# AkshayThiru/incentive-design-mpc

Hardware: AMD Instinct MI355X
Metric: LoMPC QP solves/sec (higher is better)
Workload: dtype f64

## Files before the change

incentive-design-mpc_amd/csrc/lompc_ctx.hpp:

```cpp
#pragma once
#include <hip/hip_runtime.h>
#include <stdint.h>

#include <algorithm>
#include <string>
#include <vector>

#include "lompc_qp.hpp"
#include "../../include/lompc_amd.h"

#define NPX 7
enum {
  PX_COST = 0,
  PX_PRICE0 = 1,
  PX_MAX_ERR = 2,
  PX_N_OK = 3,
  PX_N_REPAIRED = 4,
  PX_N_FAILED = 5,
  PX_N_INVALID = 6
};

struct lompc_ctx {
  int device = 0;
  int N = 0;
// ... 66 lines not shown
  int scalar_cells = 0;
  int nblk = 0;
  int n_cu = 0;
  bool close = false;
  bool close_no_w = true;
  int* d_arrive = nullptr;
  int n_empty = 0;
  CtxEnds ce{};
  int eval_occ = 1;
  int64_t eval_occ_key = -1;
  int64_t cap_S = 0, cap_blk = 0, cap_cells = 0;
  const double* gamma = nullptr;
  const double* w_ref = nullptr;
  double* d_stats_own = nullptr;
  double* d_stats = nullptr;
  int64_t* d_set_off = nullptr;
  int* d_blk_prefix = nullptr;
  int4* d_blk = nullptr;
  double* d_window = nullptr;
  unsigned long long* d_wacc = nullptr;
  double* d_partial = nullptr;
  int* d_fail_cnt = nullptr;
  int* d_fail_idx = nullptr;
  int* t_cnt = nullptr;
  double* t_lo = nullptr;
  double* t_ge = nullptr;
  double* t_cf = nullptr;
  double2* t_ab = nullptr;
  uint8_t* t_sl = nullptr;
  uint8_t* d_ws = nullptr;
  struct Stepped {
    bool ok = false;
    int nblk = 0, np_wg = 0;
    char* d_map = nullptr;
    char* h_map = nullptr;
    int64_t cap_map = 0;
    PathTab tab[2]{};
    uint8_t* sl3 = nullptr;
    int64_t cap_cells = 0;
    double* part[2] = {nullptr, nullptr};
    int* fcnt[2] = {nullptr, nullptr};
    int* fidx[2] = {nullptr, nullptr};
    int64_t cap_blk = 0;
    int occ = 0;
    int64_t occ_key = -1;
    bool wide = false;
    bool stg = false;
    PathTab wt{};
    int64_t cap_wt = 0;
    double* rpart = nullptr;
    int* rfcnt = nullptr;
    int* rfidx = nullptr;
    int64_t cap_rrec = 0;
  } stp;
  int* d_errflag = nullptr;
  unsigned long long* d_tally = nullptr;
  struct lompc_comm* comm = nullptr;
  double* d_xsend = nullptr;
  double* d_xrecv = nullptr;
  int64_t cap_xsend = 0, cap_xrecv = 0;
  const int* skip = nullptr;
  int* d_loop = nullptr;
  struct lq_host_loop* h_loop = nullptr;
  double* h_dec = nullptr;
  int cap_loop_iter = 0;
  double* d_aggrec = nullptr;
  int64_t cap_aggrec = 0;
  int64_t aggrec_zero = -1;
  bool sorted = false;
  int nsblk = 0, aggF = 0;
  int4* d_sblk = nullptr;
  int* d_sblk_prefix = nullptr;
  unsigned long long* d_bsum = nullptr;
  unsigned long long* d_P = nullptr;
  int* d_pos = nullptr;
  int4* d_sinfo = nullptr;
  int64_t cap_sblk = 0, cap_P = 0, cap_pos = 0, cap_sinfo = 0;
  char* h_buf = nullptr;
  int64_t cap_h = 0;
  int64_t reserve_B = 0;
  int64_t h_off_at = 0;
  hipEvent_t ev_stage = nullptr;
  int prof = 0;
  std::vector<hipEvent_t> prof_ev[LOMPC_PLAN_KERNELS], prof_pool;
  std::vector<int> prof_mult[LOMPC_PLAN_KERNELS];
  double prof_ms[LOMPC_PLAN_KERNELS] = {0.0, 0.0, 0.0, 0.0};
  int64_t prof_n[LOMPC_PLAN_KERNELS] = {0, 0, 0, 0};
  std::string err;
};

#define HIPCHK(obj, call)                                                        \
  do {                                                                           \
    hipError_t e__ = (call);                                                     \
    if (e__ != hipSuccess) {                                                     \
      if (obj) (obj)->err = std::string(#call) + ": " + hipGetErrorString(e__); \
      return LOMPC_ERR_HIP;                                                      \
    }                                                                            \
  } while (0)

template <typename O>
static inline int fail_arg(O* o, const char* msg) {
  if (o) o->err = msg;
  return LOMPC_ERR_INVALID_ARG;
}

template <typename O, typename T>
// ... 44 lines not shown
```

incentive-design-mpc_amd/csrc/lompc_plan.hip:

```cpp
#include <hip/hip_ext.h>
#include <hip/hip_runtime.h>
#include <stdint.h>
#include <string.h>

#include <algorithm>
#include <chrono>
#include <cmath>
#include <cstdlib>
#include <map>
#include <mutex>
#include <type_traits>
#include <utility>

#include "lompc_ctx.hpp"
#include "lompc_loopstep.hpp"
#include "lompc_wave.hpp"

#ifdef LOMPC_STAMPS
#ifdef LOMPC_STAMPS_RT
#define __builtin_amdgcn_s_memtime __builtin_amdgcn_s_memrealtime
#endif
__device__ long long g_stamps[65536 * 8];
__device__ long long g_wstart[32768 * 8];
__device__ unsigned long long g_lstamps[64 * 16];
// ... 1594 lines not shown
#if LQ_EVALS_KARGS
    typedef __attribute__((address_space(4))) const EvalArgs karg_t;
    typedef __attribute__((address_space(4))) const EvalsArgs kargx_t;
    typedef __attribute__((address_space(4))) const char kargc_t;
    karg_t* ka = (karg_t*)__builtin_amdgcn_kernarg_segment_ptr();
    asm volatile("" : "+s"(ka));
    const EvalArgs& ar = *(const EvalArgs*)ka;
    const EvalsArgs& x = *(const EvalsArgs*)(kargx_t*)((kargc_t*)ka + KARG_X);
#else
    const EvalArgs& ar = a;
    const EvalsArgs& x = x_;
#endif
    const int j = x.run0 + r;
    RunOff ro;
    ro.tab = (int64_t)(j % x.slots) * x.SG;
    ro.rec = r * x.nblk;
    ro.ev = (int64_t)j * x.ev_stride;
    ro.lmbd = ar.lmbd + (size_t)j * x.lm_stride;
    ro.lmbd_r = ar.lmbd_r + (size_t)j * x.lr_stride;
    ro.launder = true;
    ro.gamma_lds = r > 0;
    ro.pipelined = LQ_EVALS_PIPELINED;
    ro.first = r == 0;
#ifdef LQ_EVALS_NOSTAGE
    ro.nostage = r > 0;
#endif
    int bl = b;
    asm volatile("" : "+s"(bl));
#ifdef LOMPC_STAMPS
    const long long t0__ = __builtin_amdgcn_s_memtime();
#endif
    eval_block<NT, false>(ar, bl, nullptr, ro);
#if LQ_EVALS_RUN_BARRIER
    __syncthreads();
#endif
#ifdef LOMPC_STAMPS
    if (threadIdx.x == 0 && r < 32 && b < 512) {
      long long* q = g_stamps + ((size_t)b * 32 + r) * 8;
      const long long* e = g_stamps + (32768 + b) * 8;
      q[0] = t0__;
      q[1] = e[6];
      q[2] = e[0];
      q[3] = e[2];
      q[4] = e[3];
      q[5] = e[1];
      q[6] = e[4];
      q[7] = __builtin_amdgcn_s_memtime();
    }
#endif
  }
}

template <int NT>
__global__ __launch_bounds__(EVAL_EVS, EVAL_MIN_WAVES) void k_evals_st(EvalArgs a, EvalsArgs x) {
  extern __shared__ __attribute__((aligned(16))) double2 s_dyn[];
  const int b = (int)blockIdx.x, tid = (int)threadIdx.x, lane = tid & 63;
  const int wv = __builtin_amdgcn_readfirstlane(tid >> 6);
  const int N = NT ? NT : a.N, G = a.G, capc = a.cap;
  const size_t tb = ctab_bytes(N, G, capc);
  char* const base = reinterpret_cast<char*>(s_dyn);
  double* const accw = reinterpret_cast<double*>(base + 2 * tb);
  double* const red = accw + (size_t)2 * EVAL_WAVES * N;
  const int s = a.blk[b].x;
  if (wv == LQ_EVALS_RW) {
    const int NS = eval_row_stride(N);
    for (int k = 0; k < 2; ++k) {
      const CTab T = ctab_at(base + k * tb, N, G, capc);
      for (int i = lane; i < 2 * NS; i += 64) T.ab[(size_t)capc * NS + i] = make_double2(0.0, 0.0);
      for (int i = lane; i < N; i += 64) accw[((size_t)k * EVAL_WAVES + LQ_EVALS_RW) * N + i] = 0.0;
      if (lane < 8) red[((size_t)k * EVAL_WAVES + LQ_EVALS_RW) * 8 + lane] = 0.0;
    }
    stage_compact(a, s, (int64_t)(x.run0 % x.slots) * x.SG, ctab_at(base, N, G, capc), N, G, capc, lane);
  }
  __syncthreads();
  for (int r = 0; r < x.nruns; ++r) {
    const int j = x.run0 + r;
    if (wv < LQ_EVALS_RW) {
      RunOff ro;
      ro.tab = (int64_t)(j % x.slots) * x.SG;
      ro.rec = r * x.nblk;
      ro.ev = (int64_t)j * x.ev_stride;
      ro.lmbd = a.lmbd + (size_t)j * x.lm_stride;
      ro.lmbd_r = a.lmbd_r + (size_t)j * x.lr_stride;
      ro.launder = true;
      ro.gamma_lds = r > 0;
      ro.buf = r & 1;
      int bl = b;
      asm volatile("" : "+s"(bl));
      eval_block<NT, false, true>(a, bl, nullptr, ro);
    } else if (r + 1 < x.nruns) {
      stage_compact(a, s, (int64_t)((j + 1) % x.slots) * x.SG, ctab_at(base + ((r + 1) & 1) * tb, N, G, capc), N, G,
                    capc, lane);
    }
    __syncthreads();
    if (wv == 0) {
      const int rb = r * x.nblk + b;
      const int par = r & 1;
      double* part = a.partial + (size_t)rb * (N + NPX);
      for (int c = lane; c < N + NPX; c += 64) {
        double v = 0.0;
        if (c < N) {
          for (int k = 0; k < EVAL_WAVES; ++k) v += accw[((size_t)par * EVAL_WAVES + k) * N + c];
        } else {
          const int xx = c - N;
          for (int k = 0; k < EVAL_WAVES; ++k) {
            const double u = red[((size_t)par * EVAL_WAVES + k) * 8 + xx];
            v = xx == PX_MAX_ERR ? fmax(v, u) : v + u;
          }
        }
        st_wt8(part + c, v);
      }
      if (lane == 0) st_wt4(a.fail_cnt + (size_t)rb * EVAL_WAVES + LQ_EVALS_RW, 0);
    }
  }
}

typedef void (*EvalsKernel)(EvalArgs, EvalsArgs);
EvalsKernel evals_st_kernel(int N) {
  switch (N) {
    case 12: return k_evals_st<12>;
    case 16: return k_evals_st<16>;
    case 24: return k_evals_st<24>;
    case 48: return k_evals_st<48>;
    default: return k_evals_st<0>;
  }
}
EvalsKernel evals_kernel(int N) {
  switch (N) {
    case 12: return k_evals<12>;
    case 16: return k_evals<16>;
    case 24: return k_evals<24>;
    case 48: return k_evals<48>;
    default: return k_evals<0>;
  }
}

struct ClosesArgs {
  int run0, nruns, slots, nblk, S, last;
  int rel;
  int64_t lm_stride, lr_stride, ev_stride, sw_stride, st_stride, SG;
};

__global__ __launch_bounds__(256) void k_closes(FinalArgs f, ClosesArgs x) {
  __shared__ double red[LQ_FIN_CLASSES][FIN_W];
  __shared__ double rep[LQ_FIN_CLASSES][FIN_W];
  const int r = (int)blockIdx.x / x.S, s = (int)blockIdx.x - r * x.S, j = x.run0 + r, N = f.N;
  FinalArgs c = f;
  c.lmbd = f.lmbd + (size_t)j * x.lm_stride;
  c.lmbd_r = f.lmbd_r + (size_t)j * x.lr_stride;
  c.t_sl = f.t_sl + (int64_t)(j % x.slots) * x.SG * 64;
  c.partial = f.partial + (size_t)r * x.nblk * (N + NPX);
  c.fail_cnt = f.fail_cnt + (size_t)r * x.nblk * EVAL_WAVES;
  c.fail_idx = f.fail_idx + (size_t)r * x.nblk * EVAL_MAXB;
  const bool last = j == x.last;
  if (x.ev_stride) {
    const size_t eo = (size_t)j * x.ev_stride;
    if (f.w) c.w = f.w + eo * N;
    if (f.cost) c.cost = f.cost + eo;
    if (f.w0) c.w0 = f.w0 + eo;
    if (f.status) c.status = f.status + eo;
  } else if (!last) {
    c.w = c.cost = c.w0 = nullptr;
    c.status = nullptr;
  }
  const int js = x.rel ? r : j;
  if (f.set_sum_w) c.set_sum_w = (x.sw_stride || last) ? f.set_sum_w + (size_t)js * x.sw_stride : nullptr;
  if (f.set_stats) c.set_stats = (x.st_stride || last) ? f.set_stats + (size_t)js * x.st_stride : nullptr;
  if (!last) c.stats = nullptr;
  finalize_set<4, false>(c, s, red, rep);
}

#include "lompc_agg.hpp"
#include "lompc_scalar.hpp"

constexpr int LQ_LOOP_G = 16;
constexpr int LQ_LOOP_G2 = 32;

// ... 1330 lines not shown
  const int64_t rounds = std::max<int64_t>(1, (10 * B + 9ll * slots * maxb - 1) / (9ll * slots * maxb));
  const int64_t target = free1 + (rounds - 1) * slots;
  std::vector<int64_t> off(S + 1);
  {
    const int64_t* hoff = reinterpret_cast<const int64_t*>(p->h_buf + p->h_off_at);
    for (int64_t s = 0; s <= S; ++s) off[s] = hoff[s];
  }
  std::vector<int4> blks;
  std::vector<int> pre;
  block_map(off.data(), S, B, maxb, target, p->n_cu, wide && rounds == 1, blks, pre);
  int64_t nblk = (int64_t)blks.size();
  const size_t o_pre = ((size_t)nblk * sizeof(int4) + 15) & ~(size_t)15;
  const size_t bytes = o_pre + (size_t)(S + 1) * sizeof(int);
  int rc;
  if ((int64_t)bytes > z.cap_map) {
    if (z.h_map) HIPCHK(p, hipHostFree(z.h_map));
    z.h_map = nullptr;
    HIPCHK(p, hipHostMalloc((void**)&z.h_map, bytes, hipHostMallocDefault));
    if ((rc = grow(p, &z.d_map, bytes))) return rc;
    z.cap_map = (int64_t)bytes;
  }
  HIPCHK(p, hipStreamSynchronize(st));
  memcpy(z.h_map, blks.data(), (size_t)nblk * sizeof(int4));
  memcpy(z.h_map + o_pre, pre.data(), (size_t)(S + 1) * sizeof(int));
  HIPCHK(p, hipMemcpyAsync(z.d_map, z.h_map, bytes, hipMemcpyHostToDevice, st));
  z.nblk = (int)nblk;
  if (ncell > z.cap_cells) {
    for (int k = 0; k < 2; ++k) {
      auto& t = z.tab[k];
      if ((rc = grow(p, &t.cnt, ncell)) || (rc = grow(p, &t.lo, ncell)) || (rc = grow(p, &t.ge, ncell * LQ_PPL)) ||
          (rc = grow(p, &t.cf, ncell * LQ_PPL * 8)) || (rc = grow(p, &t.ab, ncell * LQ_PPL * N)))
        return rc;
    }
    if ((rc = grow(p, &z.sl3, 3 * (size_t)ncell * 64))) return rc;
    z.cap_cells = ncell;
  }
  if (nblk > z.cap_blk) {
    for (int k = 0; k < 2; ++k)
      if ((rc = grow(p, &z.part[k], (size_t)nblk * (N + NPX))) || (rc = grow(p, &z.fcnt[k], (size_t)nblk * EVAL_WAVES)) ||
          (rc = grow(p, &z.fidx[k], (size_t)nblk * EVAL_MAXB)))
        return rc;
    z.cap_blk = nblk;
  }
  z.ok = true;
  z.wide = wide;
  z.stg = stg;
  return LOMPC_OK;
}

#ifndef LQ_WIDE_RUNS
#define LQ_WIDE_RUNS 64
#endif
#define LQ_WIDE_BYTES (1ll << 30)

int64_t wide_fit(const lompc_plan* p) {
  const int64_t ncell = p->S * p->G;
  const int64_t cell_bytes = LQ_PPL * (16 * (int64_t)p->N + 8 * 8 + 8) + 4 + 8 + 64;
  return std::min<int64_t>(LQ_WIDE_BYTES / (ncell * cell_bytes), INT32_MAX / 64 / ncell) - 1;
}

int wide_ring(lompc_plan* p, hipStream_t st) {
  auto& z = p->stp;
  int rc;
  const int N = p->N;
  const int64_t ncell = p->S * p->G;
  const int64_t ring = (std::min<int64_t>(LQ_WIDE_RUNS, wide_fit(p)) + 1) * ncell;
  if (ring > z.cap_wt) {
    auto& t = z.wt;
    const int64_t c = ring;
    if ((rc = grow(p, &t.cnt, c)) || (rc = grow(p, &t.lo, c)) || (rc = grow(p, &t.ge, c * LQ_PPL)) ||
        (rc = grow(p, &t.cf, c * LQ_PPL * 8)) || (rc = grow(p, &t.ab, c * LQ_PPL * N)) || (rc = grow(p, &t.sl, c * 64)))
      return rc;
    HIPCHK(p, hipMemsetAsync(t.ge, 0, (size_t)c * LQ_PPL * sizeof(*t.ge), st));
    HIPCHK(p, hipMemsetAsync(t.cf, 0, (size_t)c * LQ_PPL * 8 * sizeof(*t.cf), st));
    HIPCHK(p, hipMemsetAsync(t.ab, 0, (size_t)c * LQ_PPL * N * sizeof(*t.ab), st));
    HIPCHK(p, hipMemsetAsync(t.sl, 0, (size_t)c * 64 * sizeof(*t.sl), st));
    z.cap_wt = c;
  }
  return LOMPC_OK;
}

int lq_run_steps_stepped(lompc_plan* p, const double* lmbd, int64_t lmbd_stride, const double* lmbd_r,
                         int64_t lmbd_r_stride, int n_runs, int profile_every, bool span_events, double* w, double* cost,
                         double* w0, int8_t* status, int64_t ev_stride, double* set_sum_w, int64_t sw_stride,
                         double* set_stats, int64_t st_stride, bool split, hipStream_t st, bool scalar = false) {
  auto& z = p->stp;
  int rc;
  const int N = p->N;
  const int64_t ncell = p->S * p->G, L = p->S * (N + LOMPC_SET_STATS);
  const int K = n_runs;
  const int64_t fit = wide_fit(p);
  const int Kc = (int)std::min<int64_t>({(int64_t)K, LQ_WIDE_RUNS, fit});
  const bool wide = (p->flags & LOMPC_PLAN_WARM_START) == 0 && Kc >= 1;
  const int slots = Kc + 1;
  if ((!z.ok || z.wide != wide || z.stg != (wide && evals_stg_ok(p))) && (rc = stepped_setup(p, st, wide))) return rc;
  const bool xr = p->comm != nullptr;
  if (xr && (rc = lq_xbufs(p, 2))) return rc;
  if (wide && (rc = wide_ring(p, st))) return rc;
  auto tab = [&](int j) {
    if (wide) {
      const int64_t o = (int64_t)(j % slots) * ncell;
      PathTab t;
      t.cnt = z.wt.cnt + o;
      t.lo = z.wt.lo + o;
      t.ge = z.wt.ge + o * LQ_PPL;
      t.cf = z.wt.cf + o * LQ_PPL * 8;
      t.ab = z.wt.ab + o * LQ_PPL * N;
      t.sl = z.wt.sl + o * 64;
      return t;
    }
    PathTab t = z.tab[j & 1];
    t.sl = z.sl3 + (size_t)(j % 3) * ncell * 64;
    return t;
  };
  auto lm = [&](int j) { return lmbd + (size_t)j * lmbd_stride; };
  auto lr = [&](int j) { return lmbd_r + (size_t)j * lmbd_r_stride; };
  auto sw_of = [&](int j) { return set_sum_w ? set_sum_w + (size_t)j * sw_stride : nullptr; };
  auto st_of = [&](int j) { return set_stats ? set_stats + (size_t)j * st_stride : nullptr; };
  auto xsend = [&](int j) { return p->d_xsend + (size_t)(j & 1) * L; };
// ... 1 lines not shown
    const size_t eo = (size_t)j * ev_stride;
    eval_args(p, lm(j), lr(j), w ? w + eo * N : nullptr, cost ? cost + eo : nullptr, w0 ? w0 + eo : nullptr,
              status ? status + eo : nullptr, tab(j), a, r);
    a.blk = reinterpret_cast<const int4*>(z.d_map);
    a.nblk = z.nblk;
    a.partial = z.part[j & 1];
    r.partial = z.part[j & 1];
    a.fail_cnt = z.fcnt[j & 1];
    r.fail_cnt = z.fcnt[j & 1];
    a.fail_idx = z.fidx[j & 1];
    r.fail_idx = z.fidx[j & 1];
    r.blk_prefix = reinterpret_cast<const int*>(z.d_map + (((size_t)z.nblk * sizeof(int4) + 15) & ~(size_t)15));
    r.set_sum_w = xr ? xsend(j) : sw_of(j);
    r.set_stats = xr ? xsend(j) + p->S * N : st_of(j);
    if (ev_stride == 0 && j != K - 1) {
      r.w = r.cost = r.w0 = nullptr;
      r.status = nullptr;
    }
  };
  const size_t lds = eval_lds(N, p->G, p->cap);
  const StepKernel kern = step_kernel(N);
  if (wide && (!split || z.stg || !w)) {
    const int64_t rec_run = (int64_t)z.nblk * ((N + NPX) * 8 + EVAL_WAVES * 4 + EVAL_MAXB * 4);
    const int64_t kr = std::max<int64_t>(1, std::min<int64_t>(std::min<int64_t>(LQ_WIDE_RUNS, fit), LQ_WIDE_BYTES / rec_run));
    const int64_t need = kr * z.nblk;
    if (need > z.cap_rrec) {
      if ((rc = grow(p, &z.rpart, need * (N + NPX))) || (rc = grow(p, &z.rfcnt, need * EVAL_WAVES)) ||
          (rc = grow(p, &z.rfidx, need * EVAL_MAXB)))
        return rc;
      HIPCHK(p, hipMemsetAsync(z.rpart, 0, (size_t)need * (N + NPX) * sizeof(*z.rpart), st));
      HIPCHK(p, hipMemsetAsync(z.rfcnt, 0, (size_t)need * EVAL_WAVES * sizeof(*z.rfcnt), st));
      HIPCHK(p, hipMemsetAsync(z.rfidx, 0, (size_t)need * EVAL_MAXB * sizeof(*z.rfidx), st));
      z.cap_rrec = need;
    }
    if (xr && (rc = lq_xbufs(p, Kc, Kc))) return rc;
    EvalArgs ea;
    FinalArgs ff;
    eval_args(p, lmbd, lmbd_r, w, cost, w0, status, tab(0), ea, ff);
    ea.piece_sums = w ? 0 : 1;
    ea.blk = reinterpret_cast<const int4*>(z.d_map);
    ea.nblk = z.nblk;
    ea.partial = z.rpart;
    ff.partial = z.rpart;
    ea.fail_cnt = z.rfcnt;
    ff.fail_cnt = z.rfcnt;
    ea.fail_idx = z.rfidx;
    ff.fail_idx = z.rfidx;
    ff.blk_prefix = reinterpret_cast<const int*>(z.d_map + (((size_t)z.nblk * sizeof(int4) + 15) & ~(size_t)15));
    ff.set_sum_w = xr ? p->d_xsend : set_sum_w;
    ff.set_stats = xr ? p->d_xsend + p->S * N : set_stats;
    const int grp = split ? 1 : (int)std::min<int64_t>(Kc, kr);
    if (z.stg) ea.cap = std::min(LQ_EVALS_CAP, p->G * LQ_PPL);
    const size_t lds_e = z.stg ? evals_st_lds(N, p->G, ea.cap) : lds;
    for (int g0 = 0; g0 < K; g0 += grp) {
      const int n = std::min(grp, K - g0);
      {
        PathArgs pw = path_args(p, lmbd, lmbd_r, z.wt);
        hipEvent_t e0 = nullptr, e1 = nullptr;
        if (plan_prof_begin(p, LOMPC_PLAN_K_PATH, &e0, &e1)) return fail_arg(p, "profiling events");
        hipExtLaunchKernelGGL(paths_kernel(N), dim3((unsigned)(n * ncell)), dim3(64), 0, st, e0, e1, 0, pw, lmbd_stride,
                              lmbd_r_stride, g0, slots);
        HIPCHK(p, hipGetLastError());
        plan_prof_end(p, LOMPC_PLAN_K_PATH, e0, e1, scalar ? n : 1);
      }
      {
        hipEvent_t e0 = nullptr, e1 = nullptr;
        const bool ev = !span_events || g0 == 0;
        const int kk = scalar ? LOMPC_PLAN_K_SCALAR : LOMPC_PLAN_K_EVAL;
        if (ev && plan_prof_begin(p, kk, &e0, &e1)) return fail_arg(p, "profiling events");
        const EvalsArgs x{g0, n, slots, z.nblk, lmbd_stride, lmbd_r_stride, ev_stride, ncell};
        if (scalar)
          hipExtLaunchKernelGGL(k_scalars, dim3((unsigned)(n * z.nblk)), dim3(EVAL_EVS), scalar_lds(p->G, p->scalar_cells), st,
                                e0, e1, 0, ea, x, p->scalar_cells, K - 1);
        else
          hipExtLaunchKernelGGL(z.stg ? evals_st_kernel(N) : evals_kernel(N), dim3((unsigned)z.nblk), dim3(EVAL_EVS), lds_e, st,
                                e0, e1, 0, ea, x);
        HIPCHK(p, hipGetLastError());
        if (ev) plan_prof_end(p, kk, e0, e1, n);
      }
      {
        hipEvent_t e0 = nullptr, e1 = nullptr;
        if (plan_prof_begin(p, LOMPC_PLAN_K_FINAL, &e0, &e1)) return fail_arg(p, "profiling events");
        const ClosesArgs c{g0, n, slots, z.nblk, (int)p->S, K - 1, xr ? 1 : 0, lmbd_stride, lmbd_r_stride, ev_stride,
                           xr ? L : sw_stride, xr ? L : st_stride, ncell};
        hipExtLaunchKernelGGL(k_closes, dim3((unsigned)(n * p->S)), dim3(256), 0, st, e0, e1, 0, ff, c);
        HIPCHK(p, hipGetLastError());
        plan_prof_end(p, LOMPC_PLAN_K_FINAL, e0, e1, n);
      }
      if (xr) {
        if ((rc = lq_comm_allgather(p->comm, p->d_xsend, p->d_xrecv, (size_t)n * L, st))) {
          p->err = p->comm->err;
          return rc;
        }
        if (set_sum_w || set_stats) {
          const CombineRunsArgs ca{p->d_xrecv, p->comm->nranks, n, (int)p->S, N, g0, K - 1, set_sum_w, set_stats,
                                   sw_stride, st_stride};
          const int64_t tot = (int64_t)n * L;
          hipLaunchKernelGGL(k_combine_runs, dim3((unsigned)std::max<int64_t>(1, std::min<int64_t>((tot + 255) / 256, 1024))),
                             dim3(256), 0, st, ca);
          HIPCHK(p, hipGetLastError());
        }
      }
    }
    return LOMPC_OK;
  }
  const int s_first = 1, s_last = wide ? Kc - 1 : K - 1;
  hipEvent_t span0 = nullptr, span1 = nullptr;
  if (span_events && s_last >= s_first && plan_prof_begin(p, LOMPC_PLAN_K_EVAL, &span0, &span1))
    return fail_arg(p, "profiling events");
  auto launch = [&](const PathArgs& pa, const EvalArgs& ea, const FinalArgs& ff, int npw, int ne, int nf, bool prof,
                    hipEvent_t s0, hipEvent_t s1) -> int {
    if (npw + ne + nf == 0) return LOMPC_OK;
    hipEvent_t e0 = s0, e1 = s1;
    if (prof && plan_prof_begin(p, LOMPC_PLAN_K_EVAL, &e0, &e1)) return fail_arg(p, "profiling events");
    hipExtLaunchKernelGGL(kern, dim3((unsigned)(npw + ne + nf)), dim3(EVAL_EVS), lds, st, e0, e1, 0, pa, ea, ff, npw, ne,
                          nf);
    HIPCHK(p, hipGetLastError());
    if (prof) plan_prof_end(p, LOMPC_PLAN_K_EVAL, e0, e1);
    return LOMPC_OK;
  };
  int paths_to = 0;
  const int last = wide ? K : K + 1;
  for (int k = 0; k <= last; ++k) {
    PathArgs pa{};
    int npw = 0;
    EvalArgs ea{}, unused_e;
    FinalArgs ff{}, unused_f;
// ... 182 lines not shown
  if (!p || n_runs < 0 || !lmbd0 || !lmbd_r || !w_target || !lmbd_out || !set_sum_w || !set_stats ||
      !(step >= 0.0) || !std::isfinite(step))
    return LOMPC_ERR_INVALID_ARG;
  HIPCHK(p, hipSetDevice(p->device));
  hipStream_t st = (hipStream_t)stream;
  const int N = p->N;
  const size_t L = (size_t)p->S * 3 * N, SN = (size_t)p->S * N, SS = (size_t)p->S * LOMPC_SET_STATS;
  for (int k = 0; k < n_runs; ++k) {
    double* lm = lmbd_out + (size_t)k * L;
    if (k == 0) {
      if (lm != lmbd0) HIPCHK(p, hipMemcpyAsync(lm, lmbd0, L * sizeof(double), hipMemcpyDeviceToDevice, st));
    } else {
      hipLaunchKernelGGL(k_chain_price, dim3((unsigned)p->S), dim3(64 * ((3 * N + 63) / 64)), 0, st, p->d_q, p->ce,
                         p->nctx, N, lm - L, set_sum_w + (k - 1) * SN, set_stats + (k - 1) * SS, w_target, step, lm);
      HIPCHK(p, hipGetLastError());
    }
    const int rc = lq_plan_launch(p, lm, lmbd_r, w, cost, w0, status, set_sum_w + k * SN, set_stats + k * SS, st, nullptr);
    if (rc) return rc;
  }
  return LOMPC_OK;
}

int lompc_plan_status(lompc_plan* p, void* stream, int64_t* n_repaired, int64_t* n_failed, int64_t* n_invalid) {
  if (!p) return LOMPC_ERR_INVALID_ARG;
  HIPCHK(p, hipSetDevice(p->device));
  unsigned long long h[3] = {0, 0, 0};
  int ef = 0;
  HIPCHK(p, hipMemcpyAsync(h, p->d_tally, sizeof(h), hipMemcpyDeviceToHost, (hipStream_t)stream));
  HIPCHK(p, hipMemcpyAsync(&ef, p->d_errflag, sizeof(int), hipMemcpyDeviceToHost, (hipStream_t)stream));
  HIPCHK(p, hipMemsetAsync(p->d_tally, 0, sizeof(h), (hipStream_t)stream));
  HIPCHK(p, hipStreamSynchronize((hipStream_t)stream));
  if (n_repaired) *n_repaired = (int64_t)h[0];
  if (n_failed) *n_failed = (int64_t)h[1];
  if (n_invalid) *n_invalid = (int64_t)h[2];
  if (h[1]) p->err = lq_failed_text(p, (hipStream_t)stream);
  if (ef) {
    HIPCHK(p, hipMemsetAsync(p->d_errflag, 0, sizeof(int), (hipStream_t)stream));
    return fail_arg(p, "negative or NaN price parameter (lmbd >= 0, lmbd_r >= 0 required)");
  }
  return LOMPC_OK;
}

int lompc_plan_get_info(const lompc_plan* p, int64_t* B, int64_t* S, int* cells, int* eval_workgroups,
                        int* steps_group) {
  if (!p) return LOMPC_ERR_INVALID_ARG;
  if (steps_group) *steps_group = p->stp.ok ? (p->stp.stg ? 2 : 1) : 0;
  if (B) *B = p->B;
  if (S) *S = p->S;
  if (cells) *cells = p->G;
  if (eval_workgroups) *eval_workgroups = p->nblk;
  return LOMPC_OK;
}

int lompc_plan_profile_enable(lompc_plan* p, int kernel_mask) {
  if (!p) return LOMPC_ERR_INVALID_ARG;
  HIPCHK(p, hipSetDevice(p->device));
  p->prof = kernel_mask & ((1 << LOMPC_PLAN_KERNELS) - 1);
  while (p->prof && p->prof_pool.size() < 512) {
    hipEvent_t e;
    HIPCHK(p, hipEventCreateWithFlags(&e, hipEventDisableSystemFence));
    p->prof_pool.push_back(e);
  }
  return LOMPC_OK;
}

int lompc_plan_profile_read(lompc_plan* p, int kernel, double* total_ms, int64_t* launches, int reset) {
  if (!p) return LOMPC_ERR_INVALID_ARG;
  if (kernel < 0 || kernel >= LOMPC_PLAN_KERNELS) return fail_arg(p, "profile_read: kernel out of range");
  HIPCHK(p, hipSetDevice(p->device));
  for (int k = 0; k < LOMPC_PLAN_KERNELS; ++k)
    if (plan_events_read(p->prof_ev[k], p->prof_mult[k], p->prof_pool, p->prof_ms[k], p->prof_n[k])) return LOMPC_ERR_HIP;
  if (total_ms) *total_ms = p->prof_ms[kernel];
  if (launches) *launches = p->prof_n[kernel];
  if (reset) {
    p->prof_ms[kernel] = 0.0;
    p->prof_n[kernel] = 0;
  }
  return LOMPC_OK;
}

const char* lompc_plan_last_error(const lompc_plan* p) { return p ? p->err.c_str() : ""; }

int lompc_plan_set_comm(lompc_plan* p, lompc_comm* comm) {
  if (!p) return LOMPC_ERR_INVALID_ARG;
  if (comm && comm->device != p->device) return fail_arg(p, "set_comm: the communicator's device differs from the plan's");
  p->comm = comm;
  return LOMPC_OK;
}

int lompc_combine_records(const double* recv, int nranks, int64_t S, int N, double* set_sum_w, double* set_stats,
                          int device, void* stream) {
  if (!recv || nranks < 1 || S < 1 || N < 1 || N > LOMPC_MAX_N || S * (N + LOMPC_SET_STATS) >= (1ll << 31))
    return LOMPC_ERR_INVALID_ARG;
  if (hipSetDevice(device) != hipSuccess) return LOMPC_ERR_HIP;
  lq_combine(recv, nranks, S, N, set_sum_w, set_stats, (hipStream_t)stream);
  return hipGetLastError() == hipSuccess ? LOMPC_OK : LOMPC_ERR_HIP;
}

int lompc_plan_destroy(lompc_plan* p) {
  lq_plan_free(p);
  return LOMPC_OK;
}

}

extern "C" int lompc_debug_plan_tables(lompc_plan* p, int* cnt, double* lo, double* ge, int* pos, int* sinfo,
// ... 13 lines not shown
```

incentive-design-mpc_amd/lompc_amd/_lib.py:

```python
from __future__ import annotations

import ctypes
import os
import threading

_HERE = os.path.dirname(os.path.abspath(__file__))
LIB_PATH = os.path.join(_HERE, "liblompc_amd.so")
if os.environ.get("LOMPC_LIB"):
    LIB_PATH = os.path.join(_HERE, os.path.basename(os.environ["LOMPC_LIB"]))

LOMPC_OK = 0
LOMPC_ERR_INVALID_ARG = 1
LOMPC_ERR_NOT_CONVERGED = 2
LOMPC_ERR_HIP = 3
LOMPC_ERR_UNSUPPORTED = 4

LOMPC_EV_SMALL = 0
LOMPC_EV_LARGE = 1
LOMPC_MODE_PATH = 0
LOMPC_MODE_DIRECT = 1
LOMPC_PLAN_MAX_CTX = 4
LOMPC_PLAN_K_PATH = 0
LOMPC_PLAN_K_EVAL = 1
LOMPC_PLAN_K_FINAL = 2
# ... 14 lines not shown
def LOMPC_PLAN_CELLS(g: int) -> int:
    return int(g) << LOMPC_PLAN_CELLS_SHIFT


LOMPC_QP_OK = 0
LOMPC_QP_REPAIRED = 1
LOMPC_QP_FAILED = 2
LOMPC_QP_INVALID = 3

LOMPC_STAT_COUNT = 0
LOMPC_STAT_SUM_W0 = 1
LOMPC_STAT_SUM_PRICE0 = 2
LOMPC_STAT_MAX_ERR = 3
LOMPC_STAT_SUM_COST = 4
LOMPC_STAT_N_REPAIRED = 5
LOMPC_STAT_N_FAILED = 6
LOMPC_STAT_N_INVALID = 7
LOMPC_SET_STATS = 8
LOMPC_MAX_N = 64

_P = ctypes.c_void_p
_D = ctypes.c_double
_I = ctypes.c_int
_L = ctypes.c_int64
SIGNATURES = [
    ("lompc_create", _I, [_I, _D, _D, _D, _D, _I, _I, ctypes.POINTER(_P)]),
    ("lompc_destroy", _I, [_P]),
    ("lompc_set_mode", _I, [_P, _I]),
    ("lompc_set_params", _I, [_P, _L, _P, _P, _P, _P, _P]),
    ("lompc_solve_batch", _I, [_P, _L, _P, _P, _P, _P, _P, _P, _P, _P, _P]),
    ("lompc_run", _I, [_P, _L, _P, _P, _P, _P, _L, _P, _P, _P, _P, _P, _P, _P, _P, _P]),
    ("lompc_solve_host", _I, [_P, _P, _D, _D, _P, _P]),
    ("lompc_last_status", _I, [_P, _P, _P, _P, _P]),
    ("lompc_profile_enable", _I, [_P, _I]),
    ("lompc_profile_read", _I, [_P, _P, _P, _I]),
    ("lompc_get_info", _I, [_P, _P, _P]),
    ("lompc_status_string", ctypes.c_char_p, [_I]),
    ("lompc_last_error", ctypes.c_char_p, [_P]),
    ("lompc_abi_version", _I, []),
    ("lompc_price_step", _I, [_I, _I, _D, _D, _D, _D, _D, _P, _P, _P, _P, _P, _P]),
    ("lompc_price_regularize", _I, [_I, _I, _D, _D, _P, _P, _P, _P]),
    ("lompc_lp_separable", _I, [_I, _I, _P, _P, _P, _P]),
    ("lompc_lp_solve", _I, [_I, _I, _P, _P, _P, _P, _P]),
    ("lompc_bimpc_solve", _I, [_I, _I, _I] + [_D] * 10 + [_P] * 6 + [_D] + [_P] * 6),
    ("lompc_plan_create", _I, [_I, _P, _P, _L, _P, _P, _P, _I, _P, ctypes.POINTER(_P)]),
    ("lompc_plan_run", _I, [_P, _P, _P, _P, _P, _P, _P, _P, _P, _P]),
    ("lompc_plan_run_steps", _I, [_P, _P, _L, _P, _L, _I, _I, _P, _P, _P, _P, _P, _P, _L, _L, _L, _I, _P]),
    ("lompc_plan_run_chain", _I, [_P, _P, _P, _P, _D, _I, _P, _P, _P, _P, _P, _P, _P, _P]),
    ("lompc_levels_layout", _I, [_P, _L, _P, _I, _P, _P, _P, _P, ctypes.POINTER(ctypes.c_size_t), _P]),
    ("lompc_levels_gamma", _I, [_P, _L, _P, _I, _D, _I, _P, _P, _P]),
    ("lompc_levels_stats", _I, [_P, _L, _P, _I, _P, _P, ctypes.POINTER(ctypes.c_size_t), _P]),
    ("lompc_plan_status", _I, [_P, _P, _P, _P, _P]),
    ("lompc_plan_get_info", _I, [_P, _P, _P, _P, _P, _P]),
    ("lompc_plan_update", _I, [_P, _L, _P, _P, _P, _P]),
    ("lompc_plan_reserve", _I, [_P, _L]),
    ("lompc_price_loop", _I, [_P, _P, _P, _P, _P, _P, _P, _P, _P, _P]),
    ("lompc_price_chain", _I, [_I, _P, _P, _P, _P]),
    ("lompc_plan_profile_enable", _I, [_P, _I]),
    ("lompc_plan_profile_read", _I, [_P, _I, _P, _P, _I]),
    ("lompc_plan_last_error", ctypes.c_char_p, [_P]),
    ("lompc_plan_destroy", _I, [_P]),
    ("lompc_comm_get_unique_id", _I, [_P]),
    ("lompc_comm_create", _I, [_P, _I, _I, _I, ctypes.POINTER(_P)]),
    ("lompc_comm_destroy", _I, [_P]),
    ("lompc_plan_set_comm", _I, [_P, _P]),
    ("lompc_combine_records", _I, [_P, _I, _L, _I, _P, _P, _I, _P]),
]
LOMPC_COMM_ID_BYTES = 128
LOMPC_LOOP_PROF_ITERS = 0
LOMPC_LOOP_PROF_WALL = 1
LOMPC_LOOP_PROF_ISSUE = 2
LOMPC_LOOP_PROF_WAIT = 3
LOMPC_LOOP_PROF_GPU = 4
LOMPC_LOOP_PROF_STEP = 5
LOMPC_LOOP_PROF_HOST = 6
LOMPC_LOOP_PROF = 8
LOMPC_LOOP_AHEAD = 2
LOMPC_BIMPC_WEIGHTED = 0
LOMPC_BIMPC_UNWEIGHTED = 1
LOMPC_BIMPC_EXP_UNWEIGHTED = 2
LOMPC_BIMPC_INFO = 5
ABI_VERSION = 5


class PriceLoopArgs(ctypes.Structure):
    _fields_ = [("N", ctypes.c_int), ("r", ctypes.c_int), ("max_iter", ctypes.c_int), ("tol_avg", ctypes.c_int),
                ("theta", ctypes.c_double), ("w_max", ctypes.c_double), ("m", ctypes.c_double),
                ("kappa", ctypes.c_double), ("eps_reg", ctypes.c_double), ("tol", ctypes.c_double),
                ("n_evs", ctypes.c_double), ("lmbd_r", ctypes.c_double),
                ("A_bar", ctypes.c_void_p), ("w_ref", ctypes.c_void_p), ("dev_in", ctypes.c_void_p),
                ("host_in", ctypes.c_void_p), ("dev_sw", ctypes.c_void_p), ("dev_st", ctypes.c_void_p),
                ("host_sw", ctypes.c_void_p), ("host_st", ctypes.c_void_p), ("prof", ctypes.c_void_p),
                ("device_loop", ctypes.c_int)]

class PriceChainPart(ctypes.Structure):
    _fields_ = [("plan", ctypes.c_void_p), ("n_evs", ctypes.c_double), ("tol", ctypes.c_double),
                ("w_ref", ctypes.c_void_p), ("dev_sw", ctypes.c_void_p), ("dev_st", ctypes.c_void_p),
                ("lmbd", ctypes.c_void_p), ("w_k", ctypes.c_void_p), ("dec_actual", ctypes.c_void_p),
                ("dec_pred", ctypes.c_void_p), ("iterations", ctypes.c_int), ("calls", ctypes.c_int),
                ("rc", ctypes.c_int), ("pad", ctypes.c_int), ("price_before_reg", ctypes.c_double),
                ("price_after_reg", ctypes.c_double)]


_lock = threading.Lock()
_lib = None

# ... 28 lines not shown
```

incentive-design-mpc_amd/lompc_amd/lompc.py:

```python
from __future__ import annotations

import ctypes
from dataclasses import dataclass

import numpy as np

from . import _lib
from .settings import MAX_BAT_CHARGE_RATE, MAX_MAX_BAT_SOC, MIN_MAX_BAT_SOC, LOMPC_MODE


class SolverError(Exception):
    """Counterpart of ``cvxpy.error.SolverError``: no certified optimum."""


@dataclass
class LoMPCConstants:

    delta: float
    theta: float
    y_max: float
    w_max: float
    ev_type: str


# ... 302 lines not shown
            if bool((gamma > ymax_ev).any()):
                raise AssertionError("gamma <= y_max required")
            if bool(torch.logical_not(gamma >= 0).any()):
                raise ValueError("Parameter value must be nonnegative.")
        if getattr(self, "sort_sets", False) and B > 0:
            g = gamma.to(torch.float64)
            o1 = torch.sort(g, stable=True).indices
            sid = torch.repeat_interleave(torch.arange(S, device=g.device),
                                          torch.as_tensor(np.diff(off), device=g.device))
            o2 = torch.sort(sid[o1], stable=True).indices
            gamma = g[o1[o2]].contiguous()
        self.gamma, self.off = gamma, off
        self.w_ref = None if w_ref is None else lo._dev(w_ref).reshape(S, N)
        wt = self._want
        per_ev = wt["w"] or wt["cost"] or wt["w0"] or wt["status"]
        if getattr(self, "S", None) != S or (per_ev and getattr(self, "B", None) != B):
            dev = f"cuda:{lo.device}"
            e = lambda shape, dt=torch.float64: torch.empty(shape, dtype=dt, device=dev)
            self.out = {
                "w": e((B, N)) if wt["w"] else None,
                "cost": e((B,)) if wt["cost"] else None,
                "w0": e((B,)) if wt["w0"] else None,
                "status": e((B,), torch.int8) if wt["status"] else None,
                "set_sum_w": e((S, N)) if wt["set"] and not getattr(self, "scalar_pass", False) else None,
                "set_stats": e((S, _lib.LOMPC_SET_STATS)) if wt["set"] else None,
            }
            self._outs = [_ptr(self.out[k]) for k in ("w", "cost", "w0", "status", "set_sum_w", "set_stats")]
        self.S, self.B = S, B
        if self.direct:
            self._args = [_ptr(self.w_ref), _ptr(self.gamma_ref), B, _ptr(self.gamma), self.off.ctypes.data] + \
                self._outs + [self._stream]

    def launches_per_run(self) -> int:
        if self.direct:
            return 2
        if self._flags & _lib.LOMPC_PLAN_SORTED_GAMMA and not any(self._want[k] for k in ("w", "cost", "w0", "status")):
            return 2 + (2 if self.comm is not None else 0)
        if self.scalar_pass and self.comm is None and self.B > 0 and not self._flags & _lib.LOMPC_PLAN_DIAG_REPAIR \
                and any(self._want[k] for k in ("cost", "w0", "status", "set")):
            return 3
        close = bool(self._flags & _lib.LOMPC_PLAN_CLOSE_IN_EVAL) or (
            not self._want["w"] and not self._flags & _lib.LOMPC_PLAN_CLOSE_IN_FINALIZE)
        return (2 if close else 3) + (2 if self.comm is not None else 0)

    def set_comm(self, comm) -> "BatchPlan":
        if self.direct:
            raise ValueError("set_comm: PATH-mode plans only")
        self._check_rc(self._lib.lompc_plan_set_comm(self._plan, None if comm is None else comm.handle))
        self.comm = comm
        return self

    def info(self) -> dict:
        if self.direct:
            return {"B": self.B, "sets": self.S, "cells": 0, "workgroups": 0, "steps_group": 0, "evals_staged": False}
        B, S, cells, wg, grp = ctypes.c_int64(0), ctypes.c_int64(0), ctypes.c_int(0), ctypes.c_int(0), ctypes.c_int(0)
        self._check_rc(self._lib.lompc_plan_get_info(self._plan, ctypes.byref(B), ctypes.byref(S), ctypes.byref(cells),
                                                     ctypes.byref(wg), ctypes.byref(grp)))
        return {"B": B.value, "sets": S.value, "cells": cells.value, "workgroups": wg.value,
                "steps_group": min(grp.value, 1), "evals_staged": grp.value == 2}

    def update(self, gamma, set_offsets, w_ref=None, validate=True) -> "BatchPlan":
        old = (self.gamma, self.w_ref, getattr(self, "out", None))
        self._layout(gamma, set_offsets, w_ref, validate)
        if not self.direct:
            rc = self._lib.lompc_plan_update(self._plan, self.B, _ptr(self.gamma), self.off.ctypes.data,
                                             _ptr(self.w_ref), self._stream)
            if rc != _lib.LOMPC_OK:
                self._broken = (old, _lib.status_text(self._lib, None, rc, plan=self._plan))
                self._check_rc(rc)
        return self

    def reserve(self, max_B: int) -> "BatchPlan":
        if not self.direct:
            self._check_rc(self._lib.lompc_plan_reserve(self._plan, int(max_B)))
            self.update(self.gamma, self.off, self.w_ref, validate=False)
        return self

    def _usable(self) -> None:
        if getattr(self, "_broken", None):
            raise RuntimeError(f"BatchPlan unusable after a failed update: {self._broken[1]}")
        if self.comm is not None and self.comm.handle is None:
            raise RuntimeError("BatchPlan: its communicator was closed; attach another (set_comm) or None")

    def __del__(self):
        if getattr(self, "_plan", None) is not None:
            try:
                self._lib.lompc_plan_destroy(self._plan)
            except Exception:
                pass
            self._plan = None

    def _check_rc(self, rc: int) -> None:
        if rc == _lib.LOMPC_OK:
            return
        text = _lib.status_text(self._lib, None, rc, plan=self._plan)
        if rc == _lib.LOMPC_ERR_INVALID_ARG:
            raise ValueError(text)
        if rc == _lib.LOMPC_ERR_NOT_CONVERGED:
            raise SolverError(text)
        raise RuntimeError(text)

    def run(self, lmbd, lmbd_r) -> dict:
        pl = lmbd if isinstance(lmbd, int) else lmbd.data_ptr()
        pr = lmbd_r if isinstance(lmbd_r, int) else lmbd_r.data_ptr()
        self._usable()
        if self.direct:
            lo = self.lompc
            rc = lo._lib.lompc_run(lo._ctx, self.S, pl, pr, *self._args)
            if rc:
                lo._check_rc(rc)
            lo.S = self.S
            return self.out
# ... 131 lines not shown
```

include/lompc_amd.h:

```cpp
#ifndef LOMPC_AMD_H
#define LOMPC_AMD_H

#include <stdint.h>

#ifdef __cplusplus
extern "C" {
#endif

#define LOMPC_OK                0
#define LOMPC_ERR_INVALID_ARG   1
#define LOMPC_ERR_NOT_CONVERGED 2
#define LOMPC_ERR_HIP           3
#define LOMPC_ERR_UNSUPPORTED   4

#define LOMPC_EV_SMALL 0
#define LOMPC_EV_LARGE 1

#define LOMPC_MODE_PATH   0
#define LOMPC_MODE_DIRECT 1

#define LOMPC_QP_OK        0
#define LOMPC_QP_REPAIRED  1
#define LOMPC_QP_FAILED    2
#define LOMPC_QP_INVALID   3
// ... 53 lines not shown
int lompc_abi_version(void);

typedef struct lompc_plan lompc_plan;
#define LOMPC_PLAN_MAX_CTX 4
#define LOMPC_PLAN_WARM_START 1
#define LOMPC_PLAN_DIAG_REPAIR 2
#define LOMPC_PLAN_CLOSE_IN_EVAL 8
#define LOMPC_PLAN_SORTED_GAMMA 16
#define LOMPC_PLAN_CLOSE_IN_FINALIZE 32
#define LOMPC_PLAN_SCALAR_PASS 64
#define LOMPC_PLAN_CELLS_SHIFT 20
#define LOMPC_PLAN_CELLS(g) ((int)(g) << LOMPC_PLAN_CELLS_SHIFT)

int lompc_plan_create(int n_ctx, lompc_ctx* const* ctxs, const int64_t* sets_per_ctx,
                      int64_t B, const double* gamma, const int64_t* set_offsets,
                      const double* w_ref, int flags, void* stream, lompc_plan** out);

int lompc_plan_update(lompc_plan* plan, int64_t B, const double* gamma, const int64_t* set_offsets,
                      const double* w_ref, void* stream);

int lompc_plan_reserve(lompc_plan* plan, int64_t max_B);

int lompc_plan_run(lompc_plan* plan, const double* lmbd, const double* lmbd_r, double* w,
                   double* cost, double* w0, int8_t* status, double* set_sum_w,
                   double* set_stats, void* stream);

#define LOMPC_STEPS_PER_KERNEL 1
#define LOMPC_STEPS_SPAN_EVENTS 2
#define LOMPC_STEPS_SCALAR_PASS 4
int lompc_plan_run_steps(lompc_plan* plan, const double* lmbd, int64_t lmbd_stride,
                         const double* lmbd_r, int64_t lmbd_r_stride, int n_runs,
                         int profile_every, double* w, double* cost, double* w0, int8_t* status,
                         double* set_sum_w, double* set_stats, int64_t set_sum_w_stride,
                         int64_t set_stats_stride, int64_t ev_stride, int steps_flags, void* stream);

int lompc_plan_run_chain(lompc_plan* plan, const double* lmbd0, const double* lmbd_r, const double* w_target,
                         double step, int n_runs, double* lmbd_out, double* w, double* cost, double* w0,
                         int8_t* status, double* set_sum_w, double* set_stats, void* stream);

int lompc_levels_layout(const double* y, int64_t n, const double* bounds, int P, double* ys, int64_t* perm,
                        double* stats, void* work, size_t* work_bytes, void* stream);

int lompc_levels_gamma(const double* ys, int64_t n, const int64_t* runs, int P, double y_max, int central,
                       const double* gsc, double* gam, void* stream);

int lompc_levels_stats(const double* y, int64_t n, const double* bounds, int P, double* stats, void* work,
                       size_t* work_bytes, void* stream);

int lompc_plan_status(lompc_plan* plan, void* stream, int64_t* n_repaired,
                      int64_t* n_failed, int64_t* n_invalid);

int lompc_plan_get_info(const lompc_plan* plan, int64_t* B, int64_t* S, int* cells, int* eval_workgroups,
                        int* steps_group);

#define LOMPC_PLAN_K_PATH 0
#define LOMPC_PLAN_K_EVAL 1
#define LOMPC_PLAN_K_FINAL 2
#define LOMPC_PLAN_K_SCALAR 3
#define LOMPC_PLAN_KERNELS 4
int lompc_plan_profile_enable(lompc_plan* plan, int kernel_mask);
int lompc_plan_profile_read(lompc_plan* plan, int kernel, double* total_ms, int64_t* launches, int reset);

const char* lompc_plan_last_error(const lompc_plan* plan);
int lompc_plan_destroy(lompc_plan* plan);

typedef struct lompc_comm lompc_comm;
#define LOMPC_COMM_ID_BYTES 128

int lompc_comm_get_unique_id(unsigned char* id);
int lompc_comm_create(const unsigned char* id, int nranks, int rank, int device, lompc_comm** out);
int lompc_comm_destroy(lompc_comm* comm);
int lompc_plan_set_comm(lompc_plan* plan, lompc_comm* comm);
int lompc_combine_records(const double* recv, int nranks, int64_t S, int N, double* set_sum_w,
                          double* set_stats, int device, void* stream);

#define LOMPC_LOOP_PROF_ITERS  0
#define LOMPC_LOOP_PROF_WALL   1
#define LOMPC_LOOP_PROF_ISSUE  2
#define LOMPC_LOOP_PROF_WAIT   3
#define LOMPC_LOOP_PROF_GPU    4
#define LOMPC_LOOP_PROF_STEP   5
#define LOMPC_LOOP_PROF_HOST   6
#define LOMPC_LOOP_PROF 8
typedef struct lompc_price_loop_args {
  int N, r, max_iter, tol_avg;
  double theta, w_max, m, kappa, eps_reg, tol, n_evs, lmbd_r;
  const double* A_bar;
  const double* w_ref;
  double* dev_in; double* host_in;
  const double* dev_sw; const double* dev_st;
  double* host_sw; double* host_st;
  double* prof;
  int device_loop;
} lompc_price_loop_args;
#define LOMPC_LOOP_AHEAD 2
int lompc_price_loop(lompc_plan* plan, const lompc_price_loop_args* args, double* lmbd, double* w_k,
                     double* dual_cost, double* dec_actual, double* dec_pred, int* iterations,
                     double* errs, void* stream);

typedef struct lompc_price_chain_part {
  lompc_plan* plan;
  double n_evs, tol;
  const double* w_ref;
  const double* dev_sw; const double* dev_st;
  double* lmbd; double* w_k; double* dec_actual; double* dec_pred;
  int iterations, calls, rc, pad;
// ... 37 lines not shown
```

Before: 23.37 billion.

## Fuse next group's path construction into the wide evals kernel launch

Adds a k_evals_tail kernel. Its first nblk workgroups evaluate the current run group, and the extra workgroups build the path tables for the next group at the same time. The wide ring buffer is doubled to 2*grp slots so the two groups do not overlap, and the separate path launch is then issued only once, for the first group. This is meant to remove one kernel launch per group and overlap path building with evaluation. In exchange it uses more ring memory, and the fused kernel may pay an occupancy cost. A counter and an info API are added for diagnostics.

```diff
diff --git a/incentive-design-mpc_amd/csrc/lompc_ctx.hpp b/incentive-design-mpc_amd/csrc/lompc_ctx.hpp
--- a/incentive-design-mpc_amd/csrc/lompc_ctx.hpp
+++ b/incentive-design-mpc_amd/csrc/lompc_ctx.hpp
@@ -142,6 +142,7 @@
     int* rfcnt = nullptr;
     int* rfidx = nullptr;
     int64_t cap_rrec = 0;
+    int64_t tail_launches = 0;
   } stp;
   int* d_errflag = nullptr;
   unsigned long long* d_tally = nullptr;
diff --git a/incentive-design-mpc_amd/csrc/lompc_plan.hip b/incentive-design-mpc_amd/csrc/lompc_plan.hip
--- a/incentive-design-mpc_amd/csrc/lompc_plan.hip
+++ b/incentive-design-mpc_amd/csrc/lompc_plan.hip
@@ -1670,6 +1670,71 @@
 }
 
 template <int NT>
+__device__ __forceinline__ void evals_runs(const EvalArgs& a, const EvalsArgs& x_, const int b) {
+  for (int r = 0; r < x_.nruns; ++r) {
+#if LQ_EVALS_KARGS
+    typedef __attribute__((address_space(4))) const EvalArgs karg_t;
+    typedef __attribute__((address_space(4))) const EvalsArgs kargx_t;
+    typedef __attribute__((address_space(4))) const char kargc_t;
+    karg_t* ka = (karg_t*)__builtin_amdgcn_kernarg_segment_ptr();
+    asm volatile("" : "+s"(ka));
+    const EvalArgs& ar = *(const EvalArgs*)ka;
+    const EvalsArgs& x = *(const EvalsArgs*)(kargx_t*)((kargc_t*)ka + KARG_X);
+#else
+    const EvalArgs& ar = a;
+    const EvalsArgs& x = x_;
+#endif
+    const int j = x.run0 + r;
+    RunOff ro;
+    ro.tab = (int64_t)(j % x.slots) * x.SG;
+    ro.rec = r * x.nblk;
+    ro.ev = (int64_t)j * x.ev_stride;
+    ro.lmbd = ar.lmbd + (size_t)j * x.lm_stride;
+    ro.lmbd_r = ar.lmbd_r + (size_t)j * x.lr_stride;
+    ro.launder = true;
+    ro.gamma_lds = r > 0;
+    ro.pipelined = LQ_EVALS_PIPELINED;
+    ro.first = r == 0;
+    int bl = b;
+    asm volatile("" : "+s"(bl));
+    eval_block<NT, false>(ar, bl, nullptr, ro);
+#if LQ_EVALS_RUN_BARRIER
+    __syncthreads();
+#endif
+  }
+}
+
+#ifndef LQ_TAIL_RUNS
+#define LQ_TAIL_RUNS (EVAL_WAVES / LQ_STEP_CELLS)
+#endif
+static_assert(LQ_TAIL_RUNS >= 1 && LQ_TAIL_RUNS * LQ_STEP_CELLS <= EVAL_WAVES, "k_evals_tail: one path per wave");
+template <int NT>
+__global__ __launch_bounds__(EVAL_EVS, EVAL_MIN_WAVES) void k_evals_tail(EvalArgs a, EvalsArgs x_, PathArgs pa, int run0p,
+                                                                          int np) {
+  const int q = (int)blockIdx.x - x_.nblk;
+  if (q < 0) {
+    evals_runs<NT>(a, x_, (int)blockIdx.x);
+    return;
+  }
+  const int wv = (int)(threadIdx.x >> 6), wr = wv / LQ_STEP_CELLS;
+  const int SG = (int)x_.SG, wpr = SG / LQ_STEP_CELLS;
+  const int r = q / wpr * LQ_TAIL_RUNS + wr, cell = (q % wpr) * LQ_STEP_CELLS + (wv - wr * LQ_STEP_CELLS);
+  if (wr >= LQ_TAIL_RUNS || r >= np) return;
+  const int j = run0p + r;
+  const int64_t o = (int64_t)(j % x_.slots) * SG;
+  PathArgs b = pa;
+  b.lmbd = pa.lmbd + (size_t)j * x_.lm_stride;
+  b.lmbd_r = pa.lmbd_r + (size_t)j * x_.lr_stride;
+  b.t_cnt = pa.t_cnt + o;
+  b.t_lo = pa.t_lo + o;
+  b.t_sl = pa.t_sl + o * 64;
+  b.t_ge = pa.t_ge + o * LQ_PPL;
+  b.t_cf = pa.t_cf + o * LQ_PPL * 8;
+  b.t_ab = pa.t_ab + o * LQ_PPL * pa.N;
+  path_cell<NT, true>(b, cell);
+}
+
+template <int NT>
 __global__ __launch_bounds__(EVAL_EVS, EVAL_MIN_WAVES) void k_evals_st(EvalArgs a, EvalsArgs x) {
   extern __shared__ __attribute__((aligned(16))) double2 s_dyn[];
   const int b = (int)blockIdx.x, tid = (int)threadIdx.x, lane = tid & 63;
@@ -1741,6 +1806,16 @@
     case 24: return k_evals_st<24>;
     case 48: return k_evals_st<48>;
     default: return k_evals_st<0>;
+  }
+}
+typedef void (*EvalsTailKernel)(EvalArgs, EvalsArgs, PathArgs, int, int);
+EvalsTailKernel evals_tail_kernel(int N) {
+  switch (N) {
+    case 12: return k_evals_tail<12>;
+    case 16: return k_evals_tail<16>;
+    case 24: return k_evals_tail<24>;
+    case 48: return k_evals_tail<48>;
+    default: return k_evals_tail<0>;
   }
 }
 EvalsKernel evals_kernel(int N) {
@@ -3177,11 +3252,18 @@
 #define LQ_WIDE_RUNS 64
 #endif
 #define LQ_WIDE_BYTES (1ll << 30)
+#ifndef LQ_WIDE_TAIL_PATHS
+#define LQ_WIDE_TAIL_PATHS 1
+#endif
 
 int64_t wide_fit(const lompc_plan* p) {
   const int64_t ncell = p->S * p->G;
   const int64_t cell_bytes = LQ_PPL * (16 * (int64_t)p->N + 8 * 8 + 8) + 4 + 8 + 64;
   return std::min<int64_t>(LQ_WIDE_BYTES / (ncell * cell_bytes), INT32_MAX / 64 / ncell) - 1;
+}
+
+int64_t wide_slots(const lompc_plan* p, int64_t grp) {
+  return LQ_WIDE_TAIL_PATHS && 2 * grp <= wide_fit(p) + 1 ? 2 * grp : grp + 1;
 }
 
 int wide_ring(lompc_plan* p, hipStream_t st) {
@@ -3189,7 +3271,7 @@
   int rc;
   const int N = p->N;
   const int64_t ncell = p->S * p->G;
-  const int64_t ring = (std::min<int64_t>(LQ_WIDE_RUNS, wide_fit(p)) + 1) * ncell;
+  const int64_t ring = wide_slots(p, std::min<int64_t>(LQ_WIDE_RUNS, wide_fit(p))) * ncell;
   if (ring > z.cap_wt) {
     auto& t = z.wt;
     const int64_t c = ring;
@@ -3297,9 +3379,13 @@
     const int grp = split ? 1 : (int)std::min<int64_t>(Kc, kr);
     if (z.stg) ea.cap = std::min(LQ_EVALS_CAP, p->G * LQ_PPL);
     const size_t lds_e = z.stg ? evals_st_lds(N, p->G, ea.cap) : lds;
+    const bool tail = LQ_WIDE_TAIL_PATHS && !split && !scalar && !z.stg && K > grp && p->G % LQ_STEP_CELLS == 0 &&
+                      wide_slots(p, grp) == 2 * (int64_t)grp && 2 * (int64_t)grp * ncell <= z.cap_wt;
+    const int slots = tail ? 2 * grp : Kc + 1;
     for (int g0 = 0; g0 < K; g0 += grp) {
       const int n = std::min(grp, K - g0);
-      {
+      const int np = tail ? std::max(0, std::min(grp, K - g0 - grp)) : 0;
+      if (!tail || g0 == 0) {
         PathArgs pw = path_args(p, lmbd, lmbd_r, z.wt);
         hipEvent_t e0 = nullptr, e1 = nullptr;
         if (plan_prof_begin(p, LOMPC_PLAN_K_PATH, &e0, &e1)) return fail_arg(p, "profiling events");
@@ -3314,10 +3400,17 @@
         const int kk = scalar ? LOMPC_PLAN_K_SCALAR : LOMPC_PLAN_K_EVAL;
         if (ev && plan_prof_begin(p, kk, &e0, &e1)) return fail_arg(p, "profiling events");
         const EvalsArgs x{g0, n, slots, z.nblk, lmbd_stride, lmbd_r_stride, ev_stride, ncell};
-        if (scalar)
+        if (scalar) {
           hipExtLaunchKernelGGL(k_scalars, dim3((unsigned)(n * z.nblk)), dim3(EVAL_EVS), scalar_lds(p->G, p->scalar_cells), st,
                                 e0, e1, 0, ea, x, p->scalar_cells, K - 1);
-        else
+        } else if (np > 0) {
+          const PathArgs pw = path_args(p, lmbd, lmbd_r, z.wt);
+          const int64_t npw = (int64_t)((np + LQ_TAIL_RUNS - 1) / LQ_TAIL_RUNS) * (ncell / LQ_STEP_CELLS);
+          hipExtLaunchKernelGGL(evals_tail_kernel(N), dim3((unsigned)(z.nblk + npw)), dim3(EVAL_EVS), lds_e, st, e0, e1, 0, ea,
+                                x, pw, g0 + grp, np);
+          if ((p->prof >> LOMPC_PLAN_K_PATH) & 1) p->prof_n[LOMPC_PLAN_K_PATH] += 1;
+          z.tail_launches += 1;
+        } else
           hipExtLaunchKernelGGL(z.stg ? evals_st_kernel(N) : evals_kernel(N), dim3((unsigned)z.nblk), dim3(EVAL_EVS), lds_e, st,
                                 e0, e1, 0, ea, x);
         HIPCHK(p, hipGetLastError());
@@ -3606,6 +3699,13 @@
   return LOMPC_OK;
 }
 
+int lompc_plan_get_wide_info(const lompc_plan* p, int64_t* ring_runs, int64_t* tail_launches) {
+  if (!p) return LOMPC_ERR_INVALID_ARG;
+  if (ring_runs) *ring_runs = std::max<int64_t>(0, wide_fit(p) + 1);
+  if (tail_launches) *tail_launches = p->stp.tail_launches;
+  return LOMPC_OK;
+}
+
 int lompc_plan_profile_enable(lompc_plan* p, int kernel_mask) {
   if (!p) return LOMPC_ERR_INVALID_ARG;
   HIPCHK(p, hipSetDevice(p->device));
diff --git a/incentive-design-mpc_amd/lompc_amd/_lib.py b/incentive-design-mpc_amd/lompc_amd/_lib.py
--- a/incentive-design-mpc_amd/lompc_amd/_lib.py
+++ b/incentive-design-mpc_amd/lompc_amd/_lib.py
@@ -90,6 +90,7 @@
     ("lompc_levels_stats", _I, [_P, _L, _P, _I, _P, _P, ctypes.POINTER(ctypes.c_size_t), _P]),
     ("lompc_plan_status", _I, [_P, _P, _P, _P, _P]),
     ("lompc_plan_get_info", _I, [_P, _P, _P, _P, _P, _P]),
+    ("lompc_plan_get_wide_info", _I, [_P, _P, _P]),
     ("lompc_plan_update", _I, [_P, _L, _P, _P, _P, _P]),
     ("lompc_plan_reserve", _I, [_P, _L]),
     ("lompc_price_loop", _I, [_P, _P, _P, _P, _P, _P, _P, _P, _P, _P]),
diff --git a/incentive-design-mpc_amd/lompc_amd/lompc.py b/incentive-design-mpc_amd/lompc_amd/lompc.py
--- a/incentive-design-mpc_amd/lompc_amd/lompc.py
+++ b/incentive-design-mpc_amd/lompc_amd/lompc.py
@@ -378,12 +378,16 @@
 
     def info(self) -> dict:
         if self.direct:
-            return {"B": self.B, "sets": self.S, "cells": 0, "workgroups": 0, "steps_group": 0, "evals_staged": False}
+            return {"B": self.B, "sets": self.S, "cells": 0, "workgroups": 0, "steps_group": 0, "evals_staged": False,
+                    "ring_runs": 0, "tail_launches": 0}
         B, S, cells, wg, grp = ctypes.c_int64(0), ctypes.c_int64(0), ctypes.c_int(0), ctypes.c_int(0), ctypes.c_int(0)
         self._check_rc(self._lib.lompc_plan_get_info(self._plan, ctypes.byref(B), ctypes.byref(S), ctypes.byref(cells),
                                                      ctypes.byref(wg), ctypes.byref(grp)))
+        ring, tail = ctypes.c_int64(0), ctypes.c_int64(0)
+        self._check_rc(self._lib.lompc_plan_get_wide_info(self._plan, ctypes.byref(ring), ctypes.byref(tail)))
         return {"B": B.value, "sets": S.value, "cells": cells.value, "workgroups": wg.value,
-                "steps_group": min(grp.value, 1), "evals_staged": grp.value == 2}
+                "steps_group": min(grp.value, 1), "evals_staged": grp.value == 2, "ring_runs": ring.value,
+                "tail_launches": tail.value}
 
     def update(self, gamma, set_offsets, w_ref=None, validate=True) -> "BatchPlan":
         old = (self.gamma, self.w_ref, getattr(self, "out", None))
diff --git a/include/lompc_amd.h b/include/lompc_amd.h
--- a/include/lompc_amd.h
+++ b/include/lompc_amd.h
@@ -129,6 +129,8 @@
 
 int lompc_plan_get_info(const lompc_plan* plan, int64_t* B, int64_t* S, int* cells, int* eval_workgroups,
                         int* steps_group);
+
+int lompc_plan_get_wide_info(const lompc_plan* plan, int64_t* ring_runs, int64_t* tail_launches);
 
 #define LOMPC_PLAN_K_PATH 0
 #define LOMPC_PLAN_K_EVAL 1
```

Result: faster. 23.78 billion, median of 6 (+1.8%).
